# nnaisense/evotorch

Hardware: NVIDIA H100
Metric: PGPE generations/sec at popsize=1Mxdim=10k (Rastrigin, fp32) (higher is better)
Workload: dtype f32

## Files before the change

evotorch_b200/csrc/evok_sample_eval.cu:

```cuda
#include <cuda.h>

#include <atomic>
#include <mutex>
#include <string>
#include <utility>
#include <vector>

#include "evok_common.cuh"

namespace evok {

struct PushArgs {
  PeerSink sink;
  const unsigned long long* epoch;
  unsigned int* done;
};


constexpr int kernel_index(int family, bool sym, bool store, bool vec) {
  return family + (sym && (family < EVOK_OBJ_KERNEL_SQ || family == EVOK_OBJ_KERNEL_BATCHED) ? 4 : 0) +
         (store && family != EVOK_OBJ_KERNEL_EVAL ? 2 : 0) + (vec ? 1 : 0);
}

constexpr int kTableKernels = EVOK_OBJ_KERNEL_BATCHED + EVOK_OBJ_BATCHED_KERNELS;
static_assert(EVOK_OBJ_KERNEL_BATCHED == EVOK_OBJ_KERNELS, "the batched family follows the first image's kernels");

static int kernel_threads(int k) { return k >= EVOK_OBJ_KERNEL_EVAL && k < EVOK_OBJ_KERNEL_BATCHED ? kEvalThreads : kSampleThreads; }

static int image_of(int k) { return k >= EVOK_OBJ_KERNEL_BATCHED ? 1 : 0; }

template <int OBJ, int V>
static void put_builtin_sampler(void** fn) {
  constexpr bool sym = V & 1, store = V & 2, vec = V & 4, push = V & 8, sq = V & 16;
  if constexpr (!(sq && (sym || push)) && (OBJ != EVOK_OBJ_NONE || (store && !push)))
    fn[kernel_index(sq ? EVOK_OBJ_KERNEL_SQ : push ? EVOK_OBJ_KERNEL_PUSH : EVOK_OBJ_KERNEL_SAMPLE, sym, store, vec)] =
        reinterpret_cast<void*>(sample_eval_kernel<ObjAcc<OBJ>, sym, store, vec, push, sq>);
}

template <int OBJ, int V>
static void put_builtin_batched(void** fn) {
  constexpr bool sym = V & 1, store = V & 2, vec = V & 4;
  if constexpr (V < EVOK_OBJ_BATCHED_KERNELS && (OBJ != EVOK_OBJ_NONE || store))
    fn[kernel_index(EVOK_OBJ_KERNEL_BATCHED, sym, store, vec)] = reinterpret_cast<void*>(sample_eval_batched_kernel<ObjAcc<OBJ>, sym, store, vec>);
}

template <int OBJ, int... V>
static void put_builtin_kernels(void** fn, std::integer_sequence<int, V...>) {
  (put_builtin_sampler<OBJ, V>(fn), ...);
  (put_builtin_batched<OBJ, V>(fn), ...);
  if constexpr (OBJ != EVOK_OBJ_NONE) {
    fn[kernel_index(EVOK_OBJ_KERNEL_EVAL, false, true, false)] = reinterpret_cast<void*>(eval_kernel<ObjAcc<OBJ>, false>);
    fn[kernel_index(EVOK_OBJ_KERNEL_EVAL, false, true, true)] = reinterpret_cast<void*>(eval_kernel<ObjAcc<OBJ>, true>);
  }
}

template <int OBJ>
static void builtin_kernels(void** fn) {
  put_builtin_kernels<OBJ>(fn, std::make_integer_sequence<int, 32>());
}

static void (*const kBuiltinKernels[EVOK_OBJ_COUNT])(void**) = {builtin_kernels<EVOK_OBJ_NONE>, builtin_kernels<EVOK_OBJ_SPHERE>,
                                                                 builtin_kernels<EVOK_OBJ_RASTRIGIN>, builtin_kernels<EVOK_OBJ_ACKLEY>};

constexpr int kMaxDevices = 64;

struct DeviceKernels {
  int state[2] = {};
  CUmodule module[2] = {};
  void* fn[kTableKernels] = {};
  int per_sm[kTableKernels] = {};
  int sms = 0;
};

struct Objective {
  std::vector<char> image[2];
  std::vector<std::string> names[2];
  int n_data = 0;
  bool is_vector[EVOK_MAX_DATA] = {};
  DeviceKernels dev[kMaxDevices];
};

struct Instance {
  int base = -1;
  const float* p[EVOK_MAX_DATA] = {};
  int64_t len[EVOK_MAX_DATA] = {}, stride[EVOK_MAX_DATA] = {};
  int64_t n_items = 1;
};

struct DriverApi {
  decltype(&cuDeviceGet) device_get = nullptr;
  decltype(&cuDeviceGetAttribute) device_attribute = nullptr;
  decltype(&cuModuleLoadData) module_load = nullptr;
  decltype(&cuModuleGetFunction) module_function = nullptr;
  decltype(&cuModuleUnload) module_unload = nullptr;
  decltype(&cuOccupancyMaxActiveBlocksPerMultiprocessor) occupancy = nullptr;
  decltype(&cuLaunchKernel) launch = nullptr;
};
static DriverApi g_driver;

template <typename F>
static bool driver_symbol(const char* name, F& fn) {
  void* p = nullptr;
  cudaDriverEntryPointQueryResult q;
  if (cudaGetDriverEntryPoint(name, &p, cudaEnableDefault, &q) != cudaSuccess || q != cudaDriverEntryPointSuccess || !p) return false;
  fn = reinterpret_cast<F>(p);
  return true;
}

static bool driver_api() {
  DriverApi& d = g_driver;
  if (d.launch) return true;
  return driver_symbol("cuDeviceGet", d.device_get) && driver_symbol("cuDeviceGetAttribute", d.device_attribute) &&
         driver_symbol("cuModuleLoadData", d.module_load) && driver_symbol("cuModuleGetFunction", d.module_function) &&
         driver_symbol("cuModuleUnload", d.module_unload) && driver_symbol("cuOccupancyMaxActiveBlocksPerMultiprocessor", d.occupancy) &&
         driver_symbol("cuLaunchKernel", d.launch);
}

static std::mutex g_objective_mutex;
static Objective g_builtin[EVOK_OBJ_COUNT];
static Objective* g_user[EVOK_OBJ_USER_CAPACITY];
static std::atomic<int> g_user_count{0};

static std::vector<Instance> g_instances;
static std::vector<int> g_free_instances;

static bool is_user(int objective) {
  return objective >= EVOK_OBJ_USER_BASE && objective - EVOK_OBJ_USER_BASE < g_user_count.load(std::memory_order_acquire);
}

static const Instance* instance_of(int objective) {
  const int64_t slot = (int64_t)objective - EVOK_OBJ_INSTANCE_BASE;
  return slot >= 0 && slot < (int64_t)g_instances.size() && g_instances[slot].base >= 0 ? &g_instances[slot] : nullptr;
}

static int base_of(int objective) {
  if (objective < EVOK_OBJ_INSTANCE_BASE) return objective;
  std::lock_guard<std::mutex> lock(g_objective_mutex);
  const Instance* inst = instance_of(objective);
  return inst ? inst->base : objective;
}

struct LaunchData {
  DataBinding binding{};
  int base = 0;
  bool vec_ok = true;
};

static int bind_data(int objective, int64_t D, int64_t items, LaunchData* out) {
  out->base = objective;
  if (objective < EVOK_OBJ_USER_BASE) return 0;
  std::lock_guard<std::mutex> lock(g_objective_mutex);
  const Instance* inst = instance_of(objective);
  if (!inst) return is_user(objective) && g_user[objective - EVOK_OBJ_USER_BASE]->n_data > 0 ? EVOK_E_NODATA : 0;
  const Objective& obj = *g_user[inst->base - EVOK_OBJ_USER_BASE];
  out->base = inst->base;
  if (inst->n_items > 1 && items != inst->n_items) return EVOK_E_BADSIZE;
  for (int i = 0; i < obj.n_data; ++i) {
    const int64_t stride = inst->n_items > 1 ? inst->stride[i] : 0;
    if (obj.is_vector[i]) {
      if (inst->len[i] != D) return EVOK_E_BADSIZE;
      if (!aligned16(inst->p[i]) || stride % 4 != 0) out->vec_ok = false;
    }
    out->binding.p[i] = inst->p[i];
    out->binding.item_stride[i] = stride;
  }
  return 0;
}

static void fill_builtin(int objective, int dev, DeviceKernels& d) {
  kBuiltinKernels[objective](d.fn);
  for (int k = 0; k < kTableKernels; ++k)
    if (d.fn[k] && (cudaOccupancyMaxActiveBlocksPerMultiprocessor(&d.per_sm[k], d.fn[k], kernel_threads(k), 0) != cudaSuccess || d.per_sm[k] <= 0))
      d.per_sm[k] = 4;
  if (cudaDeviceGetAttribute(&d.sms, cudaDevAttrMultiProcessorCount, dev) != cudaSuccess || d.sms <= 0) d.sms = kNumSMs;
  d.state[0] = d.state[1] = 1;
}

static int load_module(const Objective& obj, int part, int dev, DeviceKernels& d) {
  cudaError_t ce = cudaSetDevice(dev);
  if (ce != cudaSuccess) return (int)ce;
  if (!driver_api()) return (int)cudaErrorNotSupported;
  const DriverApi& api = g_driver;
  CUdevice cu_dev;
  CUresult r = api.device_get(&cu_dev, dev);
  if (r == CUDA_SUCCESS) r = api.device_attribute(&d.sms, CU_DEVICE_ATTRIBUTE_MULTIPROCESSOR_COUNT, cu_dev);
  if (r == CUDA_SUCCESS) r = api.module_load(&d.module[part], obj.image[part].data());
  if (r != CUDA_SUCCESS) return (int)r;
  const int k0 = part ? EVOK_OBJ_KERNEL_BATCHED : 0;
  const int n = part ? EVOK_OBJ_BATCHED_KERNELS : EVOK_OBJ_KERNELS;
  for (int i = 0; i < n; ++i) {
    const int k = k0 + i;
    CUfunction fn = nullptr;
    if (api.module_function(&fn, d.module[part], obj.names[part][i].c_str()) != CUDA_SUCCESS) {
      api.module_unload(d.module[part]);
      d.module[part] = nullptr;
      d.state[part] = EVOK_E_NOKERNEL;
      return d.state[part];
    }
    d.fn[k] = fn;
    if (api.occupancy(&d.per_sm[k], fn, kernel_threads(k), 0) != CUDA_SUCCESS || d.per_sm[k] <= 0) d.per_sm[k] = 4;
  }
  if (d.sms <= 0) d.sms = kNumSMs;
  d.state[part] = 1;
  return 0;
}

static int device_kernels(int objective, int part, const DeviceKernels** out) {
  int dev = 0;
  const cudaError_t ce = cudaGetDevice(&dev);
  if (ce != cudaSuccess) return (int)ce;
  if (dev < 0 || dev >= kMaxDevices) return EVOK_E_BADSIZE;
  std::lock_guard<std::mutex> lock(g_objective_mutex);
  const bool user = objective >= EVOK_OBJ_USER_BASE;
  Objective& obj = user ? *g_user[objective - EVOK_OBJ_USER_BASE] : g_builtin[objective];
  DeviceKernels& d = obj.dev[dev];
  if (d.state[part] == 0) {
    if (!user) fill_builtin(objective, dev, d);
    else if (obj.image[part].empty()) return EVOK_E_NOKERNEL;
    else if (const int rc = load_module(obj, part, dev, d)) return rc;
  }
  if (d.state[part] != 1) return d.state[part];
  *out = &d;
  return 0;
}

struct KernelChoice {
  int k;
  int64_t n_units;
  int64_t ctas_needed;
};

static KernelChoice choose_kernel(int family, bool sym, const float* X, int64_t ldx, const float* mu, const float* sigma, int64_t n_rows,
                                  int64_t D, const LaunchData& data, int64_t item_strides = 0) {
  const bool store = X != nullptr;
  const bool vec = (D % 4 == 0) && aligned16(mu) && aligned16(sigma) && (!store || (aligned16(X) && ldx % 4 == 0)) && item_strides % 4 == 0 &&
                   data.vec_ok;
  KernelChoice c;
  c.k = kernel_index(family, sym, store, vec);
  c.n_units = sym ? n_rows / 2 : n_rows;
  const int warps = kernel_threads(c.k) / 32;
  c.ctas_needed = (c.n_units + warps - 1) / warps;
  return c;
}

static int launch(int objective, const KernelChoice& c, void** args, cudaStream_t st, int64_t items = 1) {
  const DeviceKernels* d = nullptr;
  const int rc = device_kernels(objective, image_of(c.k), &d);
  if (rc != 0) return rc;
  int64_t g = (int64_t)d->per_sm[c.k] * d->sms / items;
  if (g > c.ctas_needed) g = c.ctas_needed;
  if (g < 1) g = 1;
  const int threads = kernel_threads(c.k);
  if (d->module[image_of(c.k)]) {
    const CUresult r = g_driver.launch(static_cast<CUfunction>(d->fn[c.k]), (unsigned)g, (unsigned)items, 1, threads, 1, 1, 0, (CUstream)st, args,
                                       nullptr);
    if (r != CUDA_SUCCESS) return (int)r;
    count_launches(1);
    return 0;
  }
  cudaLaunchKernel(d->fn[c.k], dim3((unsigned)g, (unsigned)items), dim3(threads), args, 0, st);
  EVOK_CHECK_LAUNCH();
  return 0;
}

static int check_sample(int objective, const float* X, int64_t ldx, const float* mu, const float* sigma, int64_t row0, int64_t n_rows,
                        int64_t D, bool sym, const float* f, const PushArgs* push) {
  if (!mu || !sigma) return EVOK_E_NULLPTR;
  const int first = push ? EVOK_OBJ_NONE + 1 : EVOK_OBJ_NONE;
  if ((objective < first || objective >= EVOK_OBJ_COUNT) && !is_user(objective)) return EVOK_E_BADENUM;
  if (push) {
    if (push->sink.world < 1 || push->sink.world > EVOK_MAX_PEERS || push->sink.rank < 0 || push->sink.rank >= push->sink.world)
      return EVOK_E_BADSIZE;
  } else {
    if (objective == EVOK_OBJ_NONE && !X) return EVOK_E_NULLPTR;
    if (objective != EVOK_OBJ_NONE && !f) return EVOK_E_NULLPTR;
  }
  if (n_rows < 0 || D <= 0 || row0 < 0 || (X && ldx < D)) return EVOK_E_BADSIZE;
  if (sym && ((n_rows & 1) || (row0 & 1))) return EVOK_E_ODDROWS;
  return 0;
}

static int sample(int objective, int family, float* X, int64_t ldx, const float* mu, const float* sigma, int64_t row0, int64_t n_rows,
                  int64_t D, bool sym, uint64_t seed, uint64_t stream_id, const uint32_t* stream_off, float* f, float* q, PushArgs push,
                  cudaStream_t st) {
  LaunchData data;
  if (const int rc = bind_data(objective, D, 0, &data)) return rc;
  KernelChoice c = choose_kernel(family, sym, X, ldx, mu, sigma, n_rows, D, data);
  PhiloxKey key = make_philox_key(seed, stream_id);
  void* args[] = {&X, &ldx, &mu, &sigma, &row0, &c.n_units, &D, &key, &stream_off, &f, &push.sink, &push.epoch, &push.done, &q, &data.binding};
  return launch(data.base, c, args, st);
}

}

using namespace evok;

extern "C" EVOK_API int evok_objective_register(const void* cubin, size_t bytes, const char* const* kernel_names_host, int n_kernels,
                                                int* id_out_host) {
  if (!cubin || !kernel_names_host || !id_out_host) return EVOK_E_NULLPTR;
  if (bytes == 0 || n_kernels != EVOK_OBJ_KERNELS) return EVOK_E_BADSIZE;
  for (int k = 0; k < n_kernels; ++k)
    if (!kernel_names_host[k]) return EVOK_E_NULLPTR;
  std::lock_guard<std::mutex> lock(g_objective_mutex);
  const int n = g_user_count.load(std::memory_order_relaxed);
  if (n >= EVOK_OBJ_USER_CAPACITY) return EVOK_E_BADSIZE;
  Objective* obj = new Objective;
  obj->image[0].assign(static_cast<const char*>(cubin), static_cast<const char*>(cubin) + bytes);
  for (int k = 0; k < n_kernels; ++k) obj->names[0].emplace_back(kernel_names_host[k]);
  g_user[n] = obj;
  g_user_count.store(n + 1, std::memory_order_release);
  *id_out_host = EVOK_OBJ_USER_BASE + n;
  return 0;
}

extern "C" EVOK_API int evok_objective_load(int objective) {
  objective = base_of(objective);
  if (!is_user(objective)) return EVOK_E_BADENUM;
  const DeviceKernels* d = nullptr;
  return device_kernels(objective, 0, &d);
}

extern "C" EVOK_API int evok_objective_register_batched(int objective, const void* cubin, size_t bytes, const char* const* kernel_names_host,
                                                        int n_kernels) {
  if (!cubin || !kernel_names_host) return EVOK_E_NULLPTR;
  if (bytes == 0 || n_kernels != EVOK_OBJ_BATCHED_KERNELS) return EVOK_E_BADSIZE;
  for (int k = 0; k < n_kernels; ++k)
    if (!kernel_names_host[k]) return EVOK_E_NULLPTR;
  if (!is_user(objective)) return EVOK_E_BADENUM;
  std::lock_guard<std::mutex> lock(g_objective_mutex);
  Objective& obj = *g_user[objective - EVOK_OBJ_USER_BASE];
  obj.image[1].assign(static_cast<const char*>(cubin), static_cast<const char*>(cubin) + bytes);
  obj.names[1].assign(kernel_names_host, kernel_names_host + n_kernels);
  return 0;
}

extern "C" EVOK_API int evok_objective_declare_data(int objective, int n_data, const int* is_vector_host) {
  if (!is_vector_host) return EVOK_E_NULLPTR;
  if (!is_user(objective)) return EVOK_E_BADENUM;
  if (n_data < 1 || n_data > EVOK_MAX_DATA) return EVOK_E_BADSIZE;
  std::lock_guard<std::mutex> lock(g_objective_mutex);
  Objective& obj = *g_user[objective - EVOK_OBJ_USER_BASE];
  if (obj.n_data != 0) return EVOK_E_BADSIZE;
  obj.n_data = n_data;
  for (int i = 0; i < n_data; ++i) obj.is_vector[i] = is_vector_host[i] != 0;
  return 0;
}

extern "C" EVOK_API int evok_objective_instance(int base, const float* const* ptrs_host, const int64_t* lens_host, const int64_t* item_strides_host,
                                                int64_t n_items, int n_data, int* id_out_host) {
  if (!ptrs_host || !lens_host || !item_strides_host || !id_out_host) return EVOK_E_NULLPTR;
  if (!is_user(base)) return EVOK_E_BADENUM;
  std::lock_guard<std::mutex> lock(g_objective_mutex);
  const Objective& obj = *g_user[base - EVOK_OBJ_USER_BASE];
  if (obj.n_data == 0) return EVOK_E_NODATA;
  if (n_data != obj.n_data || n_items < 1) return EVOK_E_BADSIZE;
  Instance inst;
  for (int i = 0; i < n_data; ++i) {
    if (!ptrs_host[i]) return EVOK_E_NULLPTR;
    if (lens_host[i] < 1 || (lens_host[i] == 1) == obj.is_vector[i] || item_strides_host[i] < 0) return EVOK_E_BADSIZE;
    inst.p[i] = ptrs_host[i];
    inst.len[i] = lens_host[i];
    inst.stride[i] = item_strides_host[i];
  }
  inst.base = base;
  inst.n_items = n_items;
  int slot;
  if (!g_free_instances.empty()) {
    slot = g_free_instances.back();
    g_free_instances.pop_back();
  } else {
    if (g_instances.size() >= EVOK_OBJ_INSTANCE_CAPACITY) return EVOK_E_BADSIZE;
    slot = (int)g_instances.size();
    g_instances.emplace_back();
  }
  g_instances[slot] = inst;
  *id_out_host = EVOK_OBJ_INSTANCE_BASE + slot;
  return 0;
}

extern "C" EVOK_API int evok_objective_release(int id) {
  std::lock_guard<std::mutex> lock(g_objective_mutex);
  if (!instance_of(id)) return EVOK_E_BADENUM;
  g_instances[id - EVOK_OBJ_INSTANCE_BASE] = Instance{};
  g_free_instances.push_back(id - EVOK_OBJ_INSTANCE_BASE);
  return 0;
}

extern "C" EVOK_API int evok_sample_eval(int objective, float* X, int64_t ldx, const float* mu, const float* sigma, int64_t row0,
                                int64_t n_rows, int64_t D, int symmetric, uint64_t seed, uint64_t stream_id,
                                const uint32_t* stream_offset_dev, float* f, void* stream) {
  const int rc = check_sample(base_of(objective), X, ldx, mu, sigma, row0, n_rows, D, symmetric != 0, f, nullptr);
  if (rc != 0 || n_rows == 0) return rc;
  return sample(objective, EVOK_OBJ_KERNEL_SAMPLE, X, ldx, mu, sigma, row0, n_rows, D, symmetric != 0, seed, stream_id, stream_offset_dev, f,
                nullptr, PushArgs{}, (cudaStream_t)stream);
}

extern "C" EVOK_API int evok_sample_eval_sq(int objective, float* X, int64_t ldx, const float* mu, const float* sigma, int64_t row0, int64_t n_rows,
                                            int64_t D, uint64_t seed, uint64_t stream_id, const uint32_t* stream_offset_dev, float* f, float* q,
                                            void* stream) {
  if (!q) return EVOK_E_NULLPTR;
  const int rc = check_sample(base_of(objective), X, ldx, mu, sigma, row0, n_rows, D, false, f, nullptr);
  if (rc != 0 || n_rows == 0) return rc;
  return sample(objective, EVOK_OBJ_KERNEL_SQ, X, ldx, mu, sigma, row0, n_rows, D, false, seed, stream_id, stream_offset_dev, f, q, PushArgs{},
                (cudaStream_t)stream);
}

extern "C" EVOK_API int evok_sample_eval_push(int objective, float* X, int64_t ldx, const float* mu, const float* sigma, int64_t row0, int64_t n_rows,
                                              int64_t D, int symmetric, uint64_t seed, uint64_t stream_id, const uint32_t* stream_offset_dev,
                                              int world, int rank, void* const* peer_f, void* const* peer_flags, const uint64_t* epoch_dev,
                                              uint32_t* done_dev, void* stream) {
  if (!peer_f || !peer_flags || !epoch_dev || !done_dev) return EVOK_E_NULLPTR;
  PushArgs push{};
  push.sink.world = world;
// ... 85 lines not shown
```

evotorch_b200/csrc/evok_sampler.cuh:

```cuda
#pragma once

#ifdef __CUDACC_RTC__
typedef signed char int8_t;
typedef unsigned char uint8_t;
typedef int int32_t;
typedef unsigned int uint32_t;
typedef long long int64_t;
typedef unsigned long long uint64_t;
#endif

#include "../../include/evok.h"

namespace evok {

struct PeerSink {
  void* data[EVOK_MAX_PEERS];
  unsigned long long* flags[EVOK_MAX_PEERS];
  int world, rank;
};

__device__ __forceinline__ void st_release_sys(unsigned long long* p, unsigned long long v) {
  asm volatile("st.release.sys.global.u64 [%0], %1;" ::"l"(p), "l"(v) : "memory");
}
__device__ __forceinline__ unsigned long long ld_acquire_sys(const unsigned long long* p) {
  unsigned long long v;
  asm volatile("ld.acquire.sys.global.u64 %0, [%1];" : "=l"(v) : "l"(p) : "memory");
  return v;
}

static __device__ __noinline__ void peer_signal_tail(const PeerSink& s, const unsigned long long* epoch, unsigned int* done) {
  __syncthreads();
  if (threadIdx.x == 0) {
    __threadfence_system();
    const unsigned int prev = atomicAdd(done, 1u);
    if (prev == gridDim.x - 1) {
      *done = 0;
      __threadfence_system();
      const unsigned long long e = *epoch + 1ull;
      for (int p = 0; p < s.world; ++p) st_release_sys(s.flags[p] + s.rank, e);
    }
  }
}

struct U4 {
  uint32_t x, y, z, w;
};

struct PhiloxKey {
  uint32_t k0[10], k1[10];
  uint32_t stream_lo;
};

#ifndef EVOK_PHILOX_ROUNDS
#define EVOK_PHILOX_ROUNDS 10
#endif
__device__ __forceinline__ U4 philox4x32_10(U4 c, const PhiloxKey& key) {
  constexpr uint32_t M0 = 0xD2511F53u, M1 = 0xCD9E8D57u;
#pragma unroll
  for (int r = 0; r < EVOK_PHILOX_ROUNDS; ++r) {
    const uint32_t hi0 = __umulhi(M0, c.x), lo0 = M0 * c.x;
    const uint32_t hi1 = __umulhi(M1, c.z), lo1 = M1 * c.z;
    U4 n;
    n.x = hi1 ^ c.y ^ key.k0[r];
    n.y = lo1;
    n.z = hi0 ^ c.w ^ key.k1[r];
    n.w = lo0;
    c = n;
  }
  return c;
}

__device__ __forceinline__ float sqrt_approx(float x) {
  float r;
  asm("sqrt.approx.ftz.f32 %0, %1;" : "=f"(r) : "f"(x));
  return r;
}

__device__ __forceinline__ float lg2_approx(float x) {
  float r;
  asm("lg2.approx.ftz.f32 %0, %1;" : "=f"(r) : "f"(x));
  return r;
}

__device__ __forceinline__ void box_muller(uint32_t a, uint32_t b, float& z0, float& z1) {
  const float u1 = fmaf((float)a, 2.3283064365386963e-10f, 1.1641532182693481e-10f);
  const float th = fmaf((float)b, 1.4629180792671596e-09f, 7.314590396335798e-10f);
  const float r = sqrt_approx(lg2_approx(u1) * -1.3862943611198906f);
  float s, c;
  __sincosf(th, &s, &c);
  z0 = r * c;
  z1 = r * s;
}

__device__ __forceinline__ void normals4(const PhiloxKey& key, uint32_t stream_word, uint64_t unit, uint32_t q, float z[4]) {
  U4 c;
  c.x = q;
  c.y = (uint32_t)unit;
  c.z = (uint32_t)(unit >> 32);
  c.w = stream_word;
  const U4 r = philox4x32_10(c, key);
  box_muller(r.x, r.y, z[0], z[1]);
  box_muller(r.z, r.w, z[2], z[3]);
}

__device__ __forceinline__ float warp_sum(float v) {
#pragma unroll
  for (int o = 16; o > 0; o >>= 1) v += __shfl_xor_sync(0xffffffffu, v, o);
  return v;
}
__device__ __forceinline__ double warp_sum(double v) {
#pragma unroll
  for (int o = 16; o > 0; o >>= 1) v += __shfl_xor_sync(0xffffffffu, v, o);
  return v;
}

__device__ __forceinline__ float4 ld_stream4(const float* p) {
  float4 v;
  asm volatile("ld.global.nc.L1::no_allocate.v4.f32 {%0,%1,%2,%3}, [%4];" : "=f"(v.x), "=f"(v.y), "=f"(v.z), "=f"(v.w) : "l"(p));
  return v;
}
__device__ __forceinline__ float ld_stream1(const float* p) {
  float v;
  asm volatile("ld.global.nc.L1::no_allocate.f32 %0, [%1];" : "=f"(v) : "l"(p));
  return v;
}
__device__ __forceinline__ void st_stream4(float* p, float a, float b, float c, float d) {
  asm volatile("st.global.cs.v4.f32 [%0], {%1,%2,%3,%4};" ::"l"(p), "f"(a), "f"(b), "f"(c), "f"(d) : "memory");
}
__device__ __forceinline__ void st_stream1(float* p, float a) {
  asm volatile("st.global.cs.f32 [%0], %1;" ::"l"(p), "f"(a) : "memory");
}

template <int OBJ>
struct ObjAcc;

template <>
struct ObjAcc<EVOK_OBJ_NONE> {
  __device__ __forceinline__ explicit ObjAcc(int64_t) {}
  __device__ __forceinline__ void add(float, int64_t) {}
  __device__ __forceinline__ float finish(int64_t) { return 0.f; }
};
template <>
struct ObjAcc<EVOK_OBJ_SPHERE> {
  __device__ __forceinline__ explicit ObjAcc(int64_t) {}
  float s2 = 0.f;
  __device__ __forceinline__ void add(float x, int64_t) { s2 = fmaf(x, x, s2); }
  __device__ __forceinline__ float finish(int64_t) { return warp_sum(s2); }
};
template <>
struct ObjAcc<EVOK_OBJ_RASTRIGIN> {
  __device__ __forceinline__ explicit ObjAcc(int64_t) {}
  float s2 = 0.f, sc = 0.f;
  __device__ __forceinline__ void add(float x, int64_t) {
    s2 = fmaf(x, x, s2);
    sc += __cosf(6.2831853071795865f * x);
  }
  __device__ __forceinline__ float finish(int64_t D) {
    const float a = warp_sum(s2), c = warp_sum(sc);
    return fmaf(-10.f, c, a) + 10.f * (float)D;
  }
};
template <>
struct ObjAcc<EVOK_OBJ_ACKLEY> {
  __device__ __forceinline__ explicit ObjAcc(int64_t) {}
  float s2 = 0.f, sc = 0.f;
  __device__ __forceinline__ void add(float x, int64_t) {
    s2 = fmaf(x, x, s2);
    sc += __cosf(6.2831853071795865f * x);
  }
  __device__ __forceinline__ float finish(int64_t D) {
    const float a = warp_sum(s2), c = warp_sum(sc);
    const float invD = 1.0f / (float)D;
    return -20.f * expf(-0.2f * sqrtf(a * invD)) - expf(c * invD) + 20.f + 2.718281828459045f;
  }
};

template <typename Acc>
struct SampleOnly {
  static constexpr bool value = false;
};
template <>
struct SampleOnly<ObjAcc<EVOK_OBJ_NONE>> {
  static constexpr bool value = true;
};

template <typename Acc, typename = void>
struct PairTerms {
  static constexpr bool value = false;
};
template <typename Acc>
struct PairTerms<Acc, decltype(void(Acc::kPairs))> {
  static constexpr bool value = Acc::kPairs;
};

struct DataBinding {
  const float* p[EVOK_MAX_DATA];
  int64_t item_stride[EVOK_MAX_DATA];
};
struct NoData {};

template <typename Acc, typename = void>
struct DataTerms {
  static constexpr bool value = false;
  using Arg = NoData;
};
template <typename Acc>
struct DataTerms<Acc, decltype(void(Acc::kData))> {
  static constexpr bool value = Acc::kData;
  using Arg = DataBinding;
};

template <typename Acc, typename Arg>
__device__ __forceinline__ Acc make_acc(int64_t D, const Arg& data) {
  if constexpr (DataTerms<Acc>::value) return Acc(D, data);
  else return Acc(D);
}

__device__ __forceinline__ NoData item_data(const NoData& d, int64_t) { return d; }
__device__ __forceinline__ DataBinding item_data(DataBinding d, int64_t item) {
#pragma unroll
  for (int i = 0; i < EVOK_MAX_DATA; ++i) d.p[i] += item * d.item_stride[i];
  return d;
}

template <typename Acc, int N>
struct DataCols {
  static constexpr int kSlots = Acc::kVectors > 0 ? Acc::kVectors : 1;
  float v[N][kSlots], left[kSlots];
  __device__ __forceinline__ void load4(const Acc& acc, int64_t j) {
    static_assert(N == 4, "a column group is 4 columns");
#pragma unroll
    for (int i = 0; i < Acc::kVectors; ++i) {
      const float4 t = __ldg(reinterpret_cast<const float4*>(acc.vec[i] + j));
      v[0][i] = t.x; v[1][i] = t.y; v[2][i] = t.z; v[3][i] = t.w;
    }
  }
  __device__ __forceinline__ void load1(const Acc& acc, int64_t j, int c) {
#pragma unroll
    for (int i = 0; i < Acc::kVectors; ++i) v[c][i] = __ldg(acc.vec[i] + j);
  }
  __device__ __forceinline__ void load_left(const Acc& acc, int64_t j) {
#pragma unroll
    for (int i = 0; i < Acc::kVectors; ++i) left[i] = __ldg(acc.vec[i] + j - 1);
  }
};
struct NoCols {
  template <typename Acc> __device__ __forceinline__ void load4(const Acc&, int64_t) {}
  template <typename Acc> __device__ __forceinline__ void load1(const Acc&, int64_t, int) {}
  template <typename Acc> __device__ __forceinline__ void load_left(const Acc&, int64_t) {}
};
template <typename Acc, int N, bool = DataTerms<Acc>::value>
struct ColsOf {
  using type = NoCols;
};
template <typename Acc, int N>
struct ColsOf<Acc, N, true> {
  using type = DataCols<Acc, N>;
};

template <typename Acc, typename Cols>
__device__ __forceinline__ void fold(Acc& acc, float x, int64_t j, const Cols& dc, int c) {
  if constexpr (DataTerms<Acc>::value) acc.add(x, j, dc.v[c]);
  else acc.add(x, j);
}

template <int N, typename Acc, typename Cols>
__device__ __forceinline__ void fold_pairs(Acc& acc, const float (&v)[N], int64_t j, int n_valid, float& carry, const Cols& dc) {
  const int lane = threadIdx.x & 31;
  const float rot = __shfl_sync(0xffffffffu, v[N - 1], (lane + 31) & 31);
  const float left = lane == 0 ? carry : rot;
  carry = rot;
  if (n_valid > 0 && j > 0) {
    if constexpr (DataTerms<Acc>::value) acc.add_pair(left, v[0], j - 1, dc.left, dc.v[0]);
    else acc.add_pair(left, v[0], j - 1);
  }
#pragma unroll
  for (int c = 1; c < N; ++c)
    if (c < n_valid) {
      if constexpr (DataTerms<Acc>::value) acc.add_pair(v[c - 1], v[c], j + c - 1, dc.v[c - 1], dc.v[c]);
      else acc.add_pair(v[c - 1], v[c], j + c - 1);
    }
}

#ifndef EVOK_SAMPLE_THREADS
#define EVOK_SAMPLE_THREADS 256
#endif
#ifndef EVOK_SAMPLE_MINB
#define EVOK_SAMPLE_MINB 3
#endif
#ifndef EVOK_SAMPLE_UNR
#define EVOK_SAMPLE_UNR 2
#endif
#ifndef EVOK_SAMPLEONLY_MINB
#define EVOK_SAMPLEONLY_MINB 5
#endif
#ifndef EVOK_SAMPLEONLY_UNR
#define EVOK_SAMPLEONLY_UNR 1
#endif
constexpr int kSampleThreads = EVOK_SAMPLE_THREADS;
template <typename Acc>
struct SampleTune {
  static constexpr int kUnroll = SampleOnly<Acc>::value ? EVOK_SAMPLEONLY_UNR : EVOK_SAMPLE_UNR;
  static constexpr int kMinBlocks = SampleOnly<Acc>::value ? EVOK_SAMPLEONLY_MINB : EVOK_SAMPLE_MINB;
};

template <typename Acc, bool SYM, bool STORE, bool VEC, bool SQ = false>
__device__ __forceinline__ void sample_group(const PhiloxKey& key, uint32_t sw, uint64_t unit, uint32_t q, int64_t D,
                                             const float* __restrict__ mu, const float* __restrict__ sigma, float* xp, float* xm,
                                             Acc& accp, Acc& accm, float* zsq = nullptr) {
  float z[4];
  normals4(key, sw, unit, q, z);
  const int64_t j = (int64_t)q << 2;
  typename ColsOf<Acc, 4>::type dc;
  if (VEC) {
    if (SQ) {
      *zsq = fmaf(z[0], z[0], *zsq); *zsq = fmaf(z[1], z[1], *zsq); *zsq = fmaf(z[2], z[2], *zsq); *zsq = fmaf(z[3], z[3], *zsq);
    }
    const float4 m = __ldg(reinterpret_cast<const float4*>(mu + j));
    const float4 s = __ldg(reinterpret_cast<const float4*>(sigma + j));
    const float p0 = fmaf(s.x, z[0], m.x), p1 = fmaf(s.y, z[1], m.y), p2 = fmaf(s.z, z[2], m.z), p3 = fmaf(s.w, z[3], m.w);
    if (STORE) st_stream4(xp + j, p0, p1, p2, p3);
    dc.load4(accp, j);
    fold(accp, p0, j, dc, 0); fold(accp, p1, j + 1, dc, 1); fold(accp, p2, j + 2, dc, 2); fold(accp, p3, j + 3, dc, 3);
    if (SYM) {
      const float n0 = fmaf(-s.x, z[0], m.x), n1 = fmaf(-s.y, z[1], m.y), n2 = fmaf(-s.z, z[2], m.z), n3 = fmaf(-s.w, z[3], m.w);
      if (STORE) st_stream4(xm + j, n0, n1, n2, n3);
      fold(accm, n0, j, dc, 0); fold(accm, n1, j + 1, dc, 1); fold(accm, n2, j + 2, dc, 2); fold(accm, n3, j + 3, dc, 3);
    }
  } else {
#pragma unroll
    for (int c = 0; c < 4; ++c) {
      if (j + c < D) {
        if (SQ) *zsq = fmaf(z[c], z[c], *zsq);
        const float m = __ldg(mu + j + c), s = __ldg(sigma + j + c);
        const float p = fmaf(s, z[c], m);
        if (STORE) st_stream1(xp + j + c, p);
        dc.load1(accp, j + c, c);
        fold(accp, p, j + c, dc, c);
        if (SYM) {
          const float n = fmaf(-s, z[c], m);
          if (STORE) st_stream1(xm + j + c, n);
          fold(accm, n, j + c, dc, c);
        }
      }
    }
  }
}

template <typename Acc, bool SYM, bool STORE, bool VEC, bool SQ>
__device__ __forceinline__ void sample_group_pairs(const PhiloxKey& key, uint32_t sw, uint64_t unit, uint32_t q, int64_t D,
                                                   const float* __restrict__ mu, const float* __restrict__ sigma, float* xp, float* xm,
                                                   Acc& accp, Acc& accm, float* zsq, bool active, float& carry_p, float& carry_m) {
  float p[4] = {0.f, 0.f, 0.f, 0.f}, n[4] = {0.f, 0.f, 0.f, 0.f};
  const int64_t j = (int64_t)q << 2;
  int n_valid = 0;
  typename ColsOf<Acc, 4>::type dc;
  if (active) {
    float z[4];
    normals4(key, sw, unit, q, z);
    if (VEC) {
      if (SQ) {
        *zsq = fmaf(z[0], z[0], *zsq); *zsq = fmaf(z[1], z[1], *zsq); *zsq = fmaf(z[2], z[2], *zsq); *zsq = fmaf(z[3], z[3], *zsq);
      }
      const float4 m = __ldg(reinterpret_cast<const float4*>(mu + j));
      const float4 s = __ldg(reinterpret_cast<const float4*>(sigma + j));
      p[0] = fmaf(s.x, z[0], m.x); p[1] = fmaf(s.y, z[1], m.y); p[2] = fmaf(s.z, z[2], m.z); p[3] = fmaf(s.w, z[3], m.w);
      if (STORE) st_stream4(xp + j, p[0], p[1], p[2], p[3]);
      dc.load4(accp, j);
      fold(accp, p[0], j, dc, 0); fold(accp, p[1], j + 1, dc, 1); fold(accp, p[2], j + 2, dc, 2); fold(accp, p[3], j + 3, dc, 3);
      if (SYM) {
        n[0] = fmaf(-s.x, z[0], m.x); n[1] = fmaf(-s.y, z[1], m.y); n[2] = fmaf(-s.z, z[2], m.z); n[3] = fmaf(-s.w, z[3], m.w);
        if (STORE) st_stream4(xm + j, n[0], n[1], n[2], n[3]);
        fold(accm, n[0], j, dc, 0); fold(accm, n[1], j + 1, dc, 1); fold(accm, n[2], j + 2, dc, 2); fold(accm, n[3], j + 3, dc, 3);
      }
      n_valid = 4;
    } else {
#pragma unroll
      for (int c = 0; c < 4; ++c) {
        if (j + c < D) {
          if (SQ) *zsq = fmaf(z[c], z[c], *zsq);
          const float m = __ldg(mu + j + c), s = __ldg(sigma + j + c);
          p[c] = fmaf(s, z[c], m);
          if (STORE) st_stream1(xp + j + c, p[c]);
          dc.load1(accp, j + c, c);
          fold(accp, p[c], j + c, dc, c);
          if (SYM) {
            n[c] = fmaf(-s, z[c], m);
            if (STORE) st_stream1(xm + j + c, n[c]);
            fold(accm, n[c], j + c, dc, c);
          }
        }
      }
      n_valid = D - j < 4 ? (int)(D - j) : 4;
    }
  }
  if (n_valid > 0 && j > 0) dc.load_left(accp, j);
  fold_pairs<4>(accp, p, j, n_valid, carry_p, dc);
  if (SYM) fold_pairs<4>(accm, n, j, n_valid, carry_m, dc);
}

template <typename Acc, bool SYM, bool STORE, bool VEC, bool PUSH, bool SQ>
__device__ __forceinline__ void sample_eval_unit(int lane, float* __restrict__ X, int64_t ldx, const float* __restrict__ mu,
                                                 const float* __restrict__ sigma, int64_t row0, int64_t u, int64_t D, const PhiloxKey& key, uint32_t sw,
                                                 uint32_t nq, uint64_t unit0, float* __restrict__ f, const PeerSink& sink, float* __restrict__ q_out,
                                                 const typename DataTerms<Acc>::Arg& data) {
  Acc accp = make_acc<Acc>(D, data), accm = make_acc<Acc>(D, data);
  const int64_t r = SYM ? 2 * u : u;
  float* xp = STORE ? X + r * ldx : nullptr;
  float* xm = STORE ? xp + ldx : nullptr;
  const uint64_t unit = unit0 + (uint64_t)u;
  constexpr int kSampleUnroll = SampleTune<Acc>::kUnroll;
  float zsq = 0.f;
  if constexpr (PairTerms<Acc>::value) {
    float carry_p = 0.f, carry_m = 0.f;
    uint32_t b = 0;
    for (; b + 32u * kSampleUnroll <= nq; b += 32u * kSampleUnroll) {
#pragma unroll
      for (int uu = 0; uu < kSampleUnroll; ++uu)
        sample_group_pairs<Acc, SYM, STORE, VEC, SQ>(key, sw, unit, b + 32u * uu + lane, D, mu, sigma, xp, xm, accp, accm, &zsq, true,
                                                     carry_p, carry_m);
    }
    for (; b < nq; b += 32)
      sample_group_pairs<Acc, SYM, STORE, VEC, SQ>(key, sw, unit, b + lane, D, mu, sigma, xp, xm, accp, accm, &zsq, b + lane < nq,
                                                   carry_p, carry_m);
  } else {
    uint32_t q = lane;
    if (kSampleUnroll > 1) {
      for (; q + 32u * (kSampleUnroll - 1) < nq; q += 32u * kSampleUnroll) {
#pragma unroll
        for (int uu = 0; uu < kSampleUnroll; ++uu)
          sample_group<Acc, SYM, STORE, VEC, SQ>(key, sw, unit, q + 32u * uu, D, mu, sigma, xp, xm, accp, accm, &zsq);
      }
    }
    for (; q < nq; q += 32) sample_group<Acc, SYM, STORE, VEC, SQ>(key, sw, unit, q, D, mu, sigma, xp, xm, accp, accm, &zsq);
  }
  if (SQ) {
    zsq = warp_sum(zsq);
    if (lane == 0) q_out[r] = zsq;
  }
  if (!SampleOnly<Acc>::value) {
    const float fp = accp.finish(D);
    float fm = 0.f;
    if (SYM) fm = accm.finish(D);
    if (lane == 0) {
      if (PUSH) {
        for (int p = 0; p < sink.world; ++p) {
          float* fr = static_cast<float*>(sink.data[p]) + row0 + r;
          fr[0] = fp;
          if (SYM) fr[1] = fm;
        }
      } else {
        f[r] = fp;
        if (SYM) f[r + 1] = fm;
      }
    }
  }
}

template <typename Acc, bool SYM, bool STORE, bool VEC, bool PUSH, bool SQ = false>
__global__ void __launch_bounds__(kSampleThreads, SampleTune<Acc>::kMinBlocks)
    sample_eval_kernel(float* __restrict__ X, int64_t ldx, const float* __restrict__ mu, const float* __restrict__ sigma,
                       int64_t row0, int64_t n_units, int64_t D, const __grid_constant__ PhiloxKey key, const uint32_t* __restrict__ stream_off,
                       float* __restrict__ f, const __grid_constant__ PeerSink sink, const unsigned long long* epoch, unsigned int* done,
                       float* __restrict__ q_out, const typename DataTerms<Acc>::Arg data) {
  static_assert(!(SQ && (SYM || PUSH)), "the squared norms are produced by the plain non-symmetric sampler only");
  const int lane = threadIdx.x & 31;
  const uint32_t sw = key.stream_lo + (stream_off ? __ldg(stream_off) : 0u);
  const int64_t warps_total = (int64_t)gridDim.x * (kSampleThreads / 32);
  const int64_t gw = (int64_t)blockIdx.x * (kSampleThreads / 32) + (threadIdx.x >> 5);
  const uint32_t nq = (uint32_t)((D + 3) >> 2);
  const uint64_t unit0 = (uint64_t)(SYM ? (row0 >> 1) : row0);

  for (int64_t u = gw; u < n_units; u += warps_total)
    sample_eval_unit<Acc, SYM, STORE, VEC, PUSH, SQ>(lane, X, ldx, mu, sigma, row0, u, D, key, sw, nq, unit0, f, sink, q_out, data);
  if (PUSH) peer_signal_tail(sink, epoch, done);
}

template <typename Acc, bool SYM, bool STORE, bool VEC>
__global__ void __launch_bounds__(kSampleThreads, SampleTune<Acc>::kMinBlocks)
    sample_eval_batched_kernel(float* __restrict__ X, int64_t item_stride_x, int64_t ldx, const float* __restrict__ mu, int64_t item_stride_mu,
                               const float* __restrict__ sigma, int64_t item_stride_sigma, int64_t n_units, int64_t D,
                               const __grid_constant__ PhiloxKey key, float* __restrict__ f, const typename DataTerms<Acc>::Arg data) {
  const int lane = threadIdx.x & 31;
  const int64_t item = blockIdx.y;
  if (STORE) X += item * item_stride_x;
  mu += item * item_stride_mu;
  sigma += item * item_stride_sigma;
  if (!SampleOnly<Acc>::value) f += item * (SYM ? 2 * n_units : n_units);
  const uint32_t sw = key.stream_lo + (uint32_t)item;
  const int64_t warps_total = (int64_t)gridDim.x * (kSampleThreads / 32);
  const int64_t gw = (int64_t)blockIdx.x * (kSampleThreads / 32) + (threadIdx.x >> 5);
  const uint32_t nq = (uint32_t)((D + 3) >> 2);
  const PeerSink no_sink{};
  const typename DataTerms<Acc>::Arg my_data = item_data(data, item);
  for (int64_t u = gw; u < n_units; u += warps_total)
    sample_eval_unit<Acc, SYM, STORE, VEC, false, false>(lane, X, ldx, mu, sigma, 0, u, D, key, sw, nq, 0, f, no_sink, nullptr, my_data);
}

constexpr int kEvalThreads = 256;

template <typename Acc, bool VEC>
__global__ void __launch_bounds__(kEvalThreads)
    eval_kernel(const float* __restrict__ X, int64_t ldx, int64_t n_rows, int64_t D, float* __restrict__ f,
                const typename DataTerms<Acc>::Arg data) {
  const int lane = threadIdx.x & 31;
  const int64_t warps_total = (int64_t)gridDim.x * (kEvalThreads / 32);
  const int64_t gw = (int64_t)blockIdx.x * (kEvalThreads / 32) + (threadIdx.x >> 5);
  using Cols4 = typename ColsOf<Acc, 4>::type;
  using Cols1 = typename ColsOf<Acc, 1>::type;
  for (int64_t r = gw; r < n_rows; r += warps_total) {
    Acc acc = make_acc<Acc>(D, data);
    const float* x = X + r * ldx;
    if constexpr (PairTerms<Acc>::value) {
      float carry = 0.f;
      if (VEC) {
        const int64_t nq = D >> 2;
        int64_t b = 0;
        for (; b + 128 <= nq; b += 128) {
          const int64_t q = b + lane;
          float4 g[4];
#pragma unroll
          for (int k = 0; k < 4; ++k) g[k] = ld_stream4(x + 4 * (q + 32 * k));
#pragma unroll
          for (int k = 0; k < 4; ++k) {
            const int64_t jk = 4 * (q + 32 * k);
            const float v[4] = {g[k].x, g[k].y, g[k].z, g[k].w};
            Cols4 dc;
            dc.load4(acc, jk);
            if (jk > 0) dc.load_left(acc, jk);
            fold(acc, v[0], jk, dc, 0); fold(acc, v[1], jk + 1, dc, 1); fold(acc, v[2], jk + 2, dc, 2); fold(acc, v[3], jk + 3, dc, 3);
            fold_pairs<4>(acc, v, jk, 4, carry, dc);
          }
        }
        for (; b < nq; b += 32) {
          const int64_t q = b + lane;
          const bool active = q < nq;
          const float4 a = active ? ld_stream4(x + 4 * q) : make_float4(0.f, 0.f, 0.f, 0.f);
          const float v[4] = {a.x, a.y, a.z, a.w};
          const int64_t ja = 4 * q;
          Cols4 dc;
          if (active) {
            dc.load4(acc, ja);
            if (ja > 0) dc.load_left(acc, ja);
            fold(acc, v[0], ja, dc, 0); fold(acc, v[1], ja + 1, dc, 1); fold(acc, v[2], ja + 2, dc, 2); fold(acc, v[3], ja + 3, dc, 3);
          }
          fold_pairs<4>(acc, v, ja, active ? 4 : 0, carry, dc);
        }
      } else {
        for (int64_t b = 0; b < D; b += 32) {
          const int64_t j = b + lane;
          const bool active = j < D;
          const float v[1] = {active ? ld_stream1(x + j) : 0.f};
          Cols1 dc;
          if (active) {
            dc.load1(acc, j, 0);
            if (j > 0) dc.load_left(acc, j);
            fold(acc, v[0], j, dc, 0);
          }
          fold_pairs<1>(acc, v, j, active ? 1 : 0, carry, dc);
        }
      }
    } else if (VEC) {
      const int64_t nq = D >> 2;
      int64_t q = lane;
      for (; q + 96 < nq; q += 128) {
        const float4 a = ld_stream4(x + 4 * q), b = ld_stream4(x + 4 * (q + 32)), c = ld_stream4(x + 4 * (q + 64)),
                     d = ld_stream4(x + 4 * (q + 96));
        const int64_t ja = 4 * q, jb = 4 * (q + 32), jc = 4 * (q + 64), jd = 4 * (q + 96);
        Cols4 da, db, dc, dd;
        da.load4(acc, ja); db.load4(acc, jb); dc.load4(acc, jc); dd.load4(acc, jd);
        fold(acc, a.x, ja, da, 0); fold(acc, a.y, ja + 1, da, 1); fold(acc, a.z, ja + 2, da, 2); fold(acc, a.w, ja + 3, da, 3);
        fold(acc, b.x, jb, db, 0); fold(acc, b.y, jb + 1, db, 1); fold(acc, b.z, jb + 2, db, 2); fold(acc, b.w, jb + 3, db, 3);
        fold(acc, c.x, jc, dc, 0); fold(acc, c.y, jc + 1, dc, 1); fold(acc, c.z, jc + 2, dc, 2); fold(acc, c.w, jc + 3, dc, 3);
        fold(acc, d.x, jd, dd, 0); fold(acc, d.y, jd + 1, dd, 1); fold(acc, d.z, jd + 2, dd, 2); fold(acc, d.w, jd + 3, dd, 3);
      }
      for (; q < nq; q += 32) {
        const float4 a = ld_stream4(x + 4 * q);
        const int64_t ja = 4 * q;
        Cols4 da;
        da.load4(acc, ja);
        fold(acc, a.x, ja, da, 0); fold(acc, a.y, ja + 1, da, 1); fold(acc, a.z, ja + 2, da, 2); fold(acc, a.w, ja + 3, da, 3);
      }
    } else {
      for (int64_t j = lane; j < D; j += 32) {
        Cols1 dc;
        dc.load1(acc, j, 0);
        fold(acc, ld_stream1(x + j), j, dc, 0);
      }
    }
    const float v = acc.finish(D);
    if (lane == 0) f[r] = v;
  }
}

}
```

Measured before the change: 55.24.

## Stage sampled rows in shared memory and write them out with bulk async copies

When the sample-and-evaluate kernels store the population, each warp now writes its sampled values into a per-warp shared-memory buffer. A lane then issues cp.async.bulk shared-to-global copies, replacing per-thread streaming global stores. Host launch code sets and passes the dynamic shared-memory size and uses it in occupancy queries. The aim is to offload global store traffic to the TMA bulk-copy path. In exchange it adds shared-memory pressure that may lower occupancy, warp-level waits on a single staging buffer, and alignment assumptions for bulk copies.

Measured after the change: 55.97, median of 6. 1.3% higher.

```diff
diff --git a/evotorch_b200/csrc/evok_sample_eval.cu b/evotorch_b200/csrc/evok_sample_eval.cu
--- a/evotorch_b200/csrc/evok_sample_eval.cu
+++ b/evotorch_b200/csrc/evok_sample_eval.cu
@@ -26,6 +26,15 @@
 static_assert(EVOK_OBJ_KERNEL_BATCHED == EVOK_OBJ_KERNELS, "the batched family follows the first image's kernels");
 
 static int kernel_threads(int k) { return k >= EVOK_OBJ_KERNEL_EVAL && k < EVOK_OBJ_KERNEL_BATCHED ? kEvalThreads : kSampleThreads; }
+
+static int kernel_smem(int k, bool sample_only) {
+  if (sample_only || (k >= EVOK_OBJ_KERNEL_EVAL && k < EVOK_OBJ_KERNEL_BATCHED)) return 0;
+  const int family = k >= EVOK_OBJ_KERNEL_BATCHED ? EVOK_OBJ_KERNEL_BATCHED
+                     : k >= EVOK_OBJ_KERNEL_SQ    ? EVOK_OBJ_KERNEL_SQ
+                     : k >= EVOK_OBJ_KERNEL_PUSH  ? EVOK_OBJ_KERNEL_PUSH
+                                                  : EVOK_OBJ_KERNEL_SAMPLE;
+  return ((k - family) & 3) == 3 ? kSampleStageBytes : 0;
+}
 
 static int image_of(int k) { return k >= EVOK_OBJ_KERNEL_BATCHED ? 1 : 0; }
 
@@ -69,6 +78,7 @@
   CUmodule module[2] = {};
   void* fn[kTableKernels] = {};
   int per_sm[kTableKernels] = {};
+  int smem[kTableKernels] = {};
   int sms = 0;
 };
 
@@ -94,6 +104,7 @@
   decltype(&cuModuleGetFunction) module_function = nullptr;
   decltype(&cuModuleUnload) module_unload = nullptr;
   decltype(&cuOccupancyMaxActiveBlocksPerMultiprocessor) occupancy = nullptr;
+  decltype(&cuFuncSetAttribute) func_attribute = nullptr;
   decltype(&cuLaunchKernel) launch = nullptr;
 };
 static DriverApi g_driver;
@@ -113,7 +124,7 @@
   return driver_symbol("cuDeviceGet", d.device_get) && driver_symbol("cuDeviceGetAttribute", d.device_attribute) &&
          driver_symbol("cuModuleLoadData", d.module_load) && driver_symbol("cuModuleGetFunction", d.module_function) &&
          driver_symbol("cuModuleUnload", d.module_unload) && driver_symbol("cuOccupancyMaxActiveBlocksPerMultiprocessor", d.occupancy) &&
-         driver_symbol("cuLaunchKernel", d.launch);
+         driver_symbol("cuFuncSetAttribute", d.func_attribute) && driver_symbol("cuLaunchKernel", d.launch);
 }
 
 static std::mutex g_objective_mutex;
@@ -169,9 +180,13 @@
 
 static void fill_builtin(int objective, int dev, DeviceKernels& d) {
   kBuiltinKernels[objective](d.fn);
-  for (int k = 0; k < kTableKernels; ++k)
-    if (d.fn[k] && (cudaOccupancyMaxActiveBlocksPerMultiprocessor(&d.per_sm[k], d.fn[k], kernel_threads(k), 0) != cudaSuccess || d.per_sm[k] <= 0))
+  for (int k = 0; k < kTableKernels; ++k) {
+    if (!d.fn[k]) continue;
+    const int smem = d.smem[k] = kernel_smem(k, objective == EVOK_OBJ_NONE);
+    if ((smem && cudaFuncSetAttribute(d.fn[k], cudaFuncAttributeMaxDynamicSharedMemorySize, smem) != cudaSuccess) ||
+        cudaOccupancyMaxActiveBlocksPerMultiprocessor(&d.per_sm[k], d.fn[k], kernel_threads(k), smem) != cudaSuccess || d.per_sm[k] <= 0)
       d.per_sm[k] = 4;
+  }
   if (cudaDeviceGetAttribute(&d.sms, cudaDevAttrMultiProcessorCount, dev) != cudaSuccess || d.sms <= 0) d.sms = kNumSMs;
   d.state[0] = d.state[1] = 1;
 }
@@ -198,7 +213,10 @@
       return d.state[part];
     }
     d.fn[k] = fn;
-    if (api.occupancy(&d.per_sm[k], fn, kernel_threads(k), 0) != CUDA_SUCCESS || d.per_sm[k] <= 0) d.per_sm[k] = 4;
+    const int smem = d.smem[k] = kernel_smem(k, false);
+    if ((smem && api.func_attribute(fn, CU_FUNC_ATTRIBUTE_MAX_DYNAMIC_SHARED_SIZE_BYTES, smem) != CUDA_SUCCESS) ||
+        api.occupancy(&d.per_sm[k], fn, kernel_threads(k), smem) != CUDA_SUCCESS || d.per_sm[k] <= 0)
+      d.per_sm[k] = 4;
   }
   if (d.sms <= 0) d.sms = kNumSMs;
   d.state[part] = 1;
@@ -251,14 +269,15 @@
   if (g > c.ctas_needed) g = c.ctas_needed;
   if (g < 1) g = 1;
   const int threads = kernel_threads(c.k);
+  const int smem = d->smem[c.k];
   if (d->module[image_of(c.k)]) {
-    const CUresult r = g_driver.launch(static_cast<CUfunction>(d->fn[c.k]), (unsigned)g, (unsigned)items, 1, threads, 1, 1, 0, (CUstream)st, args,
-                                       nullptr);
+    const CUresult r = g_driver.launch(static_cast<CUfunction>(d->fn[c.k]), (unsigned)g, (unsigned)items, 1, threads, 1, 1, (unsigned)smem,
+                                       (CUstream)st, args, nullptr);
     if (r != CUDA_SUCCESS) return (int)r;
     count_launches(1);
     return 0;
   }
-  cudaLaunchKernel(d->fn[c.k], dim3((unsigned)g, (unsigned)items), dim3(threads), args, 0, st);
+  cudaLaunchKernel(d->fn[c.k], dim3((unsigned)g, (unsigned)items), dim3(threads), args, (size_t)smem, st);
   EVOK_CHECK_LAUNCH();
   return 0;
 }
diff --git a/evotorch_b200/csrc/evok_sampler.cuh b/evotorch_b200/csrc/evok_sampler.cuh
--- a/evotorch_b200/csrc/evok_sampler.cuh
+++ b/evotorch_b200/csrc/evok_sampler.cuh
@@ -130,6 +130,9 @@
 __device__ __forceinline__ void st_stream1(float* p, float a) {
   asm volatile("st.global.cs.f32 [%0], %1;" ::"l"(p), "f"(a) : "memory");
 }
+__device__ __forceinline__ void st_shared4(uint32_t s, float a, float b, float c, float d) {
+  asm volatile("st.shared.v4.f32 [%0], {%1,%2,%3,%4};" ::"r"(s), "f"(a), "f"(b), "f"(c), "f"(d) : "memory");
+}
 
 template <int OBJ>
 struct ObjAcc;
@@ -304,10 +307,57 @@
   static constexpr int kMinBlocks = SampleOnly<Acc>::value ? EVOK_SAMPLEONLY_MINB : EVOK_SAMPLE_MINB;
 };
 
+#ifndef EVOK_SAMPLE_STAGE_STEPS
+#define EVOK_SAMPLE_STAGE_STEPS 8
+#endif
+#ifndef EVOK_SAMPLE_STAGE_BUFS
+#define EVOK_SAMPLE_STAGE_BUFS 1
+#endif
+constexpr int kSampleStageSteps = EVOK_SAMPLE_STAGE_STEPS;
+constexpr int kSampleStageBufs = EVOK_SAMPLE_STAGE_BUFS;
+constexpr int kSampleStageRowBytes = kSampleStageSteps * 512;
+constexpr int kSampleStageBufBytes = 2 * kSampleStageRowBytes;
+constexpr int kSampleStageWarpBytes = kSampleStageBufs * kSampleStageBufBytes;
+constexpr int kSampleStageBytes = kSampleStageWarpBytes * (kSampleThreads / 32);
+
+template <typename Acc, bool STORE, bool VEC>
+constexpr bool kStagedStores = STORE && VEC && !SampleOnly<Acc>::value;
+
+extern __shared__ __align__(128) unsigned char sample_stage_smem[];
+
+struct SampleStage {
+  uint32_t base;
+  uint32_t spans;
+
+  __device__ __forceinline__ SampleStage()
+      : base((uint32_t)__cvta_generic_to_shared(sample_stage_smem) + (threadIdx.x >> 5) * kSampleStageWarpBytes), spans(0) {}
+
+  __device__ __forceinline__ uint32_t acquire() {
+    if ((threadIdx.x & 31) == 0) asm volatile("cp.async.bulk.wait_group.read %0;" ::"n"(kSampleStageBufs - 1) : "memory");
+    __syncwarp();
+    return base + (spans % kSampleStageBufs) * kSampleStageBufBytes;
+  }
+  __device__ __forceinline__ void flush(uint32_t buf, float* xp, float* xm, uint32_t bytes) {
+    asm volatile("fence.proxy.async.shared::cta;" ::: "memory");
+    __syncwarp();
+    if ((threadIdx.x & 31) == 0) {
+      asm volatile("cp.async.bulk.global.shared::cta.bulk_group [%0], [%1], %2;" ::"l"(xp), "r"(buf), "r"(bytes) : "memory");
+      if (xm)
+        asm volatile("cp.async.bulk.global.shared::cta.bulk_group [%0], [%1], %2;" ::"l"(xm), "r"(buf + kSampleStageRowBytes), "r"(bytes)
+                     : "memory");
+      asm volatile("cp.async.bulk.commit_group;" ::: "memory");
+    }
+    ++spans;
+  }
+  __device__ __forceinline__ void drain() {
+    if ((threadIdx.x & 31) == 0) asm volatile("cp.async.bulk.wait_group.read 0;" ::: "memory");
+  }
+};
+
 template <typename Acc, bool SYM, bool STORE, bool VEC, bool SQ = false>
 __device__ __forceinline__ void sample_group(const PhiloxKey& key, uint32_t sw, uint64_t unit, uint32_t q, int64_t D,
                                              const float* __restrict__ mu, const float* __restrict__ sigma, float* xp, float* xm,
-                                             Acc& accp, Acc& accm, float* zsq = nullptr) {
+                                             uint32_t sp, uint32_t sm, Acc& accp, Acc& accm, float* zsq = nullptr) {
   float z[4];
   normals4(key, sw, unit, q, z);
   const int64_t j = (int64_t)q << 2;
@@ -319,12 +369,14 @@
     const float4 m = __ldg(reinterpret_cast<const float4*>(mu + j));
     const float4 s = __ldg(reinterpret_cast<const float4*>(sigma + j));
     const float p0 = fmaf(s.x, z[0], m.x), p1 = fmaf(s.y, z[1], m.y), p2 = fmaf(s.z, z[2], m.z), p3 = fmaf(s.w, z[3], m.w);
-    if (STORE) st_stream4(xp + j, p0, p1, p2, p3);
+    if constexpr (kStagedStores<Acc, STORE, VEC>) st_shared4(sp + 4u * (uint32_t)j, p0, p1, p2, p3);
+    else if (STORE) st_stream4(xp + j, p0, p1, p2, p3);
     dc.load4(accp, j);
     fold(accp, p0, j, dc, 0); fold(accp, p1, j + 1, dc, 1); fold(accp, p2, j + 2, dc, 2); fold(accp, p3, j + 3, dc, 3);
     if (SYM) {
       const float n0 = fmaf(-s.x, z[0], m.x), n1 = fmaf(-s.y, z[1], m.y), n2 = fmaf(-s.z, z[2], m.z), n3 = fmaf(-s.w, z[3], m.w);
-      if (STORE) st_stream4(xm + j, n0, n1, n2, n3);
+      if constexpr (kStagedStores<Acc, STORE, VEC>) st_shared4(sm + 4u * (uint32_t)j, n0, n1, n2, n3);
+      else if (STORE) st_stream4(xm + j, n0, n1, n2, n3);
       fold(accm, n0, j, dc, 0); fold(accm, n1, j + 1, dc, 1); fold(accm, n2, j + 2, dc, 2); fold(accm, n3, j + 3, dc, 3);
     }
   } else {
@@ -350,7 +402,8 @@
 template <typename Acc, bool SYM, bool STORE, bool VEC, bool SQ>
 __device__ __forceinline__ void sample_group_pairs(const PhiloxKey& key, uint32_t sw, uint64_t unit, uint32_t q, int64_t D,
                                                    const float* __restrict__ mu, const float* __restrict__ sigma, float* xp, float* xm,
-                                                   Acc& accp, Acc& accm, float* zsq, bool active, float& carry_p, float& carry_m) {
+                                                   uint32_t sp, uint32_t sm, Acc& accp, Acc& accm, float* zsq, bool active, float& carry_p,
+                                                   float& carry_m) {
   float p[4] = {0.f, 0.f, 0.f, 0.f}, n[4] = {0.f, 0.f, 0.f, 0.f};
   const int64_t j = (int64_t)q << 2;
   int n_valid = 0;
@@ -365,12 +418,12 @@
       const float4 m = __ldg(reinterpret_cast<const float4*>(mu + j));
       const float4 s = __ldg(reinterpret_cast<const float4*>(sigma + j));
       p[0] = fmaf(s.x, z[0], m.x); p[1] = fmaf(s.y, z[1], m.y); p[2] = fmaf(s.z, z[2], m.z); p[3] = fmaf(s.w, z[3], m.w);
-      if (STORE) st_stream4(xp + j, p[0], p[1], p[2], p[3]);
+      if (STORE) st_shared4(sp + 4u * (uint32_t)j, p[0], p[1], p[2], p[3]);
       dc.load4(accp, j);
       fold(accp, p[0], j, dc, 0); fold(accp, p[1], j + 1, dc, 1); fold(accp, p[2], j + 2, dc, 2); fold(accp, p[3], j + 3, dc, 3);
       if (SYM) {
         n[0] = fmaf(-s.x, z[0], m.x); n[1] = fmaf(-s.y, z[1], m.y); n[2] = fmaf(-s.z, z[2], m.z); n[3] = fmaf(-s.w, z[3], m.w);
-        if (STORE) st_stream4(xm + j, n[0], n[1], n[2], n[3]);
+        if (STORE) st_shared4(sm + 4u * (uint32_t)j, n[0], n[1], n[2], n[3]);
         fold(accm, n[0], j, dc, 0); fold(accm, n[1], j + 1, dc, 1); fold(accm, n[2], j + 2, dc, 2); fold(accm, n[3], j + 3, dc, 3);
       }
       n_valid = 4;
@@ -403,7 +456,7 @@
 __device__ __forceinline__ void sample_eval_unit(int lane, float* __restrict__ X, int64_t ldx, const float* __restrict__ mu,
                                                  const float* __restrict__ sigma, int64_t row0, int64_t u, int64_t D, const PhiloxKey& key, uint32_t sw,
                                                  uint32_t nq, uint64_t unit0, float* __restrict__ f, const PeerSink& sink, float* __restrict__ q_out,
-                                                 const typename DataTerms<Acc>::Arg& data) {
+                                                 const typename DataTerms<Acc>::Arg& data, SampleStage& stage) {
   Acc accp = make_acc<Acc>(D, data), accm = make_acc<Acc>(D, data);
   const int64_t r = SYM ? 2 * u : u;
   float* xp = STORE ? X + r * ldx : nullptr;
@@ -411,28 +464,40 @@
   const uint64_t unit = unit0 + (uint64_t)u;
   constexpr int kSampleUnroll = SampleTune<Acc>::kUnroll;
   float zsq = 0.f;
-  if constexpr (PairTerms<Acc>::value) {
-    float carry_p = 0.f, carry_m = 0.f;
-    uint32_t b = 0;
-    for (; b + 32u * kSampleUnroll <= nq; b += 32u * kSampleUnroll) {
-#pragma unroll
-      for (int uu = 0; uu < kSampleUnroll; ++uu)
-        sample_group_pairs<Acc, SYM, STORE, VEC, SQ>(key, sw, unit, b + 32u * uu + lane, D, mu, sigma, xp, xm, accp, accm, &zsq, true,
+  float carry_p = 0.f, carry_m = 0.f;
+  auto groups = [&](uint32_t g0, uint32_t g1, uint32_t sp, uint32_t sm) {
+    if constexpr (PairTerms<Acc>::value) {
+      uint32_t b = g0;
+      for (; b + 32u * kSampleUnroll <= g1; b += 32u * kSampleUnroll) {
+#pragma unroll
+        for (int uu = 0; uu < kSampleUnroll; ++uu)
+          sample_group_pairs<Acc, SYM, STORE, VEC, SQ>(key, sw, unit, b + 32u * uu + lane, D, mu, sigma, xp, xm, sp, sm, accp, accm, &zsq, true,
+                                                       carry_p, carry_m);
+      }
+      for (; b < g1; b += 32)
+        sample_group_pairs<Acc, SYM, STORE, VEC, SQ>(key, sw, unit, b + lane, D, mu, sigma, xp, xm, sp, sm, accp, accm, &zsq, b + lane < g1,
                                                      carry_p, carry_m);
-    }
-    for (; b < nq; b += 32)
-      sample_group_pairs<Acc, SYM, STORE, VEC, SQ>(key, sw, unit, b + lane, D, mu, sigma, xp, xm, accp, accm, &zsq, b + lane < nq,
-                                                   carry_p, carry_m);
+    } else {
+      uint32_t q = g0 + lane;
+      if (kSampleUnroll > 1) {
+        for (; q + 32u * (kSampleUnroll - 1) < g1; q += 32u * kSampleUnroll) {
+#pragma unroll
+          for (int uu = 0; uu < kSampleUnroll; ++uu)
+            sample_group<Acc, SYM, STORE, VEC, SQ>(key, sw, unit, q + 32u * uu, D, mu, sigma, xp, xm, sp, sm, accp, accm, &zsq);
+        }
+      }
+      for (; q < g1; q += 32) sample_group<Acc, SYM, STORE, VEC, SQ>(key, sw, unit, q, D, mu, sigma, xp, xm, sp, sm, accp, accm, &zsq);
+    }
+  };
+  if constexpr (kStagedStores<Acc, STORE, VEC>) {
+    for (uint32_t g0 = 0; g0 < nq; g0 += 32u * kSampleStageSteps) {
+      const uint32_t g1 = nq - g0 < 32u * kSampleStageSteps ? nq : g0 + 32u * kSampleStageSteps;
+      const uint32_t buf = stage.acquire();
+      groups(g0, g1, buf - 16u * g0, buf + kSampleStageRowBytes - 16u * g0);
+      stage.flush(buf, xp + 4 * (int64_t)g0, SYM ? xm + 4 * (int64_t)g0 : nullptr, 16u * (g1 - g0));
+    }
   } else {
-    uint32_t q = lane;
-    if (kSampleUnroll > 1) {
-      for (; q + 32u * (kSampleUnroll - 1) < nq; q += 32u * kSampleUnroll) {
-#pragma unroll
-        for (int uu = 0; uu < kSampleUnroll; ++uu)
-          sample_group<Acc, SYM, STORE, VEC, SQ>(key, sw, unit, q + 32u * uu, D, mu, sigma, xp, xm, accp, accm, &zsq);
-      }
-    }
-    for (; q < nq; q += 32) sample_group<Acc, SYM, STORE, VEC, SQ>(key, sw, unit, q, D, mu, sigma, xp, xm, accp, accm, &zsq);
+    groups(0, nq, 0, 0);
   }
   if (SQ) {
     zsq = warp_sum(zsq);
@@ -471,8 +536,10 @@
   const uint32_t nq = (uint32_t)((D + 3) >> 2);
   const uint64_t unit0 = (uint64_t)(SYM ? (row0 >> 1) : row0);
 
+  SampleStage stage;
   for (int64_t u = gw; u < n_units; u += warps_total)
-    sample_eval_unit<Acc, SYM, STORE, VEC, PUSH, SQ>(lane, X, ldx, mu, sigma, row0, u, D, key, sw, nq, unit0, f, sink, q_out, data);
+    sample_eval_unit<Acc, SYM, STORE, VEC, PUSH, SQ>(lane, X, ldx, mu, sigma, row0, u, D, key, sw, nq, unit0, f, sink, q_out, data, stage);
+  if constexpr (kStagedStores<Acc, STORE, VEC>) stage.drain();
   if (PUSH) peer_signal_tail(sink, epoch, done);
 }
 
@@ -493,8 +560,10 @@
   const uint32_t nq = (uint32_t)((D + 3) >> 2);
   const PeerSink no_sink{};
   const typename DataTerms<Acc>::Arg my_data = item_data(data, item);
+  SampleStage stage;
   for (int64_t u = gw; u < n_units; u += warps_total)
-    sample_eval_unit<Acc, SYM, STORE, VEC, false, false>(lane, X, ldx, mu, sigma, 0, u, D, key, sw, nq, 0, f, no_sink, nullptr, my_data);
+    sample_eval_unit<Acc, SYM, STORE, VEC, false, false>(lane, X, ldx, mu, sigma, 0, u, D, key, sw, nq, 0, f, no_sink, nullptr, my_data, stage);
+  if constexpr (kStagedStores<Acc, STORE, VEC>) stage.drain();
 }
 
 constexpr int kEvalThreads = 256;
```
